# leggedrobotics/wild_visual_navigation

Hardware: AMD Instinct MI355X
Metric: frames/sec (448x448 DINO-ViT-S/8 + seg + MLP train-step) (higher is better)
Workload: dtype fp16 + e5m2-MX-correction linears (a w = a_h w_h + 2^-12 (a_h8 w_l8 + a_l8 w_h8); ~16 significand bits per product) + f16 attention products (two-plane q in the first six blocks), fp32 accumulate / residual (<= 1e-3 parity mode)

## Files before the change

include/wvn_hip.h:

```cpp
#ifndef WVN_HIP_H
#define WVN_HIP_H
#include <stddef.h>
#ifdef __cplusplus
extern "C" {
#endif

#define WVN_MAX_DEPTH 32
#define WVN_PREC_F32 0
#define WVN_PREC_BF16 1
#define WVN_PREC_X3 2
#define WVN_PREC_FP8 3
#define WVN_PREC_F16 4

#define WVN_PREC_MIX 5

int wvn_version(void);

#define WVN_VIT_MLP_FUSED 1
#define WVN_VIT_QKV_FUSED 2
#define WVN_VIT_FUSE_ANY_SIZE 4
#define WVN_VIT_NO_PROJ_IN_MLP 8
#define WVN_VIT_NO_LN_HANDOVER 16
#define WVN_VIT_NO_A384_X3 32
#define WVN_VIT_X3_NO_A384 64
// ... 289 lines not shown
int wvn_debug_mlp_x3_frag(const void* xn, const void* xn_lo, const void* W1, const void* W1_lo, const float* b1, void* hid, void* hid_lo,
                          const void* W2p, const float* b2, float* x, int M, int F, long long* dbg1, long long* dbg2, void* stream);
int wvn_debug_gemm_n384_mx(const void* A_h, const void* A_l8, const void* A_h8, const void* Wp, const float* bias, const float* ls, float* C,
                           int ldc, int M, int K, long long* dbg, void* stream);
int wvn_debug_mlp_mx(const float* x, int ldx, const float* ln_stats, const float* ln_g, const float* ln_b, const void* W1p, const float* b1,
                     void* hid_h, void* hid_l8, void* hid_h8, const void* W2p, const float* b2, float* xout, int M, int F, long long* dbg1,
                     long long* dbg2, void* stream);
int wvn_debug_qkv_mx(const float* x, int ldx, const float* ln_stats, const float* ln_g, const float* ln_b, const void* Wp, const float* bias, void* q,
                     void* q_lo, void* k, void* vt, int heads, int npad, int ntok_s, float q_scale, int M, long long* dbg, void* stream);
int wvn_debug_f16_saturate(const float* in, void* out_f16, int n, void* stream);
int wvn_debug_attention_timing(long long* dbg);
int wvn_debug_attention_variant(int variant);
int wvn_debug_attention_planes(const void* q, const void* q_lo, const void* k, const void* vt, void* out, void* out_lo, int B, int heads,
                               int ntok, int ntok_s, int npad, int out_frag, int qsplit_form, void* stream);
int wvn_debug_n384_pair(int on);
int wvn_debug_kmeans_assign_form(int form);
int wvn_debug_kmeans_linear_rows(int rows);

int wvn_debug_kmeans_screen_stats(unsigned long long* out, int reset);
int wvn_debug_qkv_fused_timing(long long* dbg);
int wvn_debug_mlp_fused_timing(long long* dbg);
int wvn_debug_gemm_n384(const void* A, int lda, const void* W, int ldw, const float* bias, float* C, int ldc, int M, int K,
                        void* stream);


size_t wvn_dense_crf_workspace_bytes(int B, int H, int W, int K);
int wvn_dense_crf(const float* logits1, int K1, long long s1b, long long s1c, long long s1p, const float* logits2, int K2, long long s2b,
                  long long s2c, long long s2p, const unsigned char* image, int B, int H, int W, int iterations, float pos_w, float pos_xy_std,
                  float bi_w, float bi_xy_std, float bi_rgb_std, int* labels, int* nseg_last, float* probs, float* debug, void* workspace,
                  size_t workspace_bytes, void* stream);
// ... 19 lines not shown
```

wild_visual_navigation_amd/_lib.py:

```python
import ctypes as C
import os
import threading

import torch

_HERE = os.path.dirname(os.path.abspath(__file__))
LIB_PATH = os.environ.get("WVN_LIB_PATH") or os.path.join(_HERE, "lib", "libwvn_hip.so")
if os.environ.get("WVN_LIB_PATH"):
    import sys as _sys

    print(f"[wild_visual_navigation_amd] WVN_LIB_PATH is set: loading {LIB_PATH} instead of the in-tree build", file=_sys.stderr)

WVN_MAX_DEPTH = 32
PREC_F32, PREC_BF16, PREC_X3, PREC_FP8, PREC_F16, PREC_MIX = 0, 1, 2, 3, 4, 5
VIT_MLP_FUSED = 1
VIT_QKV_FUSED = 2
VIT_FUSE_ANY_SIZE = 4
VIT_NO_PROJ_IN_MLP = 8
VIT_NO_LN_HANDOVER = 16
VIT_NO_A384_X3 = 32
VIT_NO_MX = 1024


def vit_qsplit_blocks(n: int) -> int:
# ... 118 lines not shown
    "wvn_slic_connectivity_scratch_bytes": ([_i, _i, _i, _i], _sz),
    "wvn_slic_connectivity": ([_p, _p, _i, _i, _i, _i, _i, _p, _sz, _p], _i),
    "wvn_seg_centers": ([_p, _p, _p, _i, _i, _i, _p], _i),
    "wvn_seg_adjacency": ([_p, _p, _p, _p, _i, _i, _i, _i, _p], _i),
    "wvn_normalize_rows": ([_p, _i, _p, _i, _i, _p], _i),
    "wvn_argmax_rows": ([_p, _i, _i, _i, _p, _p], _i),
    "wvn_kmeans_scratch_bytes": ([_i, _i, _i, _i], _sz),
    "wvn_kmeans_pixels_scratch_bytes": ([_i, _i, _i, _i, _i], _sz),
    "wvn_kmeans_cosine_pixels": ([_p, _p, _p, _p, _i, _i, _i, _i, _i, _i, _i, _p], _i),
    "wvn_flip_average": ([_p, _p, _p, _i, _i, _i, _p], _i),
    "wvn_kmeans_pixels_linear_supported_shape": ([_i, _i, _i, _i], _i),
    "wvn_kmeans_pixels_linear_scratch_bytes": ([_i, _i, _i, _i, _i], _sz),
    "wvn_kmeans_cosine_pixels_linear": ([_p, _p, _p, _p, _i, _i, _i, _i, _i, _i, _i, _p], _i),
    "wvn_debug_kmeans_linear_rows": ([_i], _i),
    "wvn_debug_n384_pair": ([_i], _i),
    "wvn_table_argmax_slots": ([_i], _i),
    "wvn_table_bilerp_argmax": ([_p, _p, _i, _i, _i, _i, _p], _i),
    "wvn_table_bilerp_argmax_ac": ([_p, _p, _i, _i, _i, _i, _i, _p], _i),
    "wvn_kmeans_cosine_pixels_linear_ac": ([_p, _p, _p, _p, _i, _i, _i, _i, _i, _i, _i, _i, _p], _i),
    "wvn_cast_rows": ([_p, _i, _p, _i, _i, _i, _i, _p], _i),
    "wvn_kmeans_cosine": ([_p, _p, _p, _p, _i, _i, _i, _i, _i, _i, _p], _i),
    "wvn_mlp_param_count": ([_p], _sz),
    "wvn_mlp_workspace_bytes": ([_p, _i], _sz),
    "wvn_double_mlp_row_tile": ([], _i),
    "wvn_double_mlp_fused_ok": ([_p, _i], _i),
    "wvn_mlp_forward": ([_p, _p, _p, _i, _i, _p, _p, _p, _p, _sz, _p], _i),
    "wvn_mlp_train_phase_a": ([_p, _p, _p, _i, _p, _i, _p, _p, _sz, _p], _i),
    "wvn_mlp_train_phase_b": ([_p, _p, _p, _i, _p, _p, _i, _p, _f, _f, _f, _p, _p, _p, _sz, _p], _i),
    "wvn_compact_segment_rows": ([_p, _i, _p, _i, _p, _i, _i, _p, _p, _p, _p], _i),
    "wvn_mlp_train_phase_a_rows": ([_p, _p, _p, _i, _p, _i, _p, _p, _p, _sz, _p, _p], _i),
# ... 67 lines not shown
```

wild_visual_navigation_amd/csrc/api.hip:

```cpp
#include <math.h>
#include <string.h>

#include "../../include/wvn_hip.h"

#include "common.h"
#include "wvn_internal.h"

#define RET_IF(x)            \
  do {                       \
    int rc__ = (x);          \
    if (rc__ != WVN_OK) return rc__; \
  } while (0)

extern "C" {

int wvn_version(void) { return 100; }

size_t wvn_vit_workspace_bytes(const wvn_vit_model* m, int batch) {
  if (!m || batch <= 0) return 0;
  return wvn_vit_workspace_bytes_impl(m, batch);
}

int wvn_vit_forward(const wvn_vit_model* m, const float* img, int batch, float* tokens_f32, void* tokens_lowp,
                    int ld_lowp, void* workspace, size_t workspace_bytes, void* stream) {
// ... 214 lines not shown
  if (!W2p) return WVN_OK;
  return wvn_gemm_n384_mx_launch(wvn_desc_n384(hid_h, hid_l8, F, W2p, nullptr, b2, nullptr, xout, 384, M, F, nullptr, dbg2, hid_h8), EPI_RESID_F32, (hipStream_t)stream);
}
int wvn_debug_qkv_mx(const float* x, int ldx, const float* ln_stats, const float* ln_g, const float* ln_b, const void* Wp, const float* bias, void* q,
                     void* q_lo, void* k, void* vt, int heads, int npad, int ntok_s, float q_scale, int M, long long* dbg, void* stream) {
  GemmBf16Params p = wvn_desc_a384(nullptr, nullptr, 0, Wp, nullptr, bias, nullptr, nullptr, 0, M, 3 * heads * 64, dbg);
  wvn_desc_ln_on_load(p, x, ldx, ln_stats, ln_g, ln_b);
  wvn_desc_qkv_epilogue(p, q, k, vt, heads, npad, 0, ntok_s, q_scale, 1, q_lo);
  return wvn_gemm_a384_mx_launch(p, EPI_QKV, (hipStream_t)stream);
}
int wvn_debug_n384_pair(int on) {
  if (on >= 32) { wvn_gemm_a384_mx_set_form(on - 32); return WVN_OK; }
  wvn_gemm_n384_x3_set_pair(on);
  return WVN_OK;
}
int wvn_debug_kmeans_screen_stats(unsigned long long* out, int reset) { return out ? wvn_kmeans_pixels_screen_stats(out, reset) : WVN_ERR_ARG; }
int wvn_debug_kmeans_assign_form(int form) { wvn_kmeans_pixels_set_assign_form(form); return WVN_OK; }
int wvn_debug_attention_variant(int v) { wvn_attention_bf16_set_variant(v); wvn_attention_bf16_set_variant_f16(v); return WVN_OK; }
int wvn_debug_attention_planes(const void* q, const void* q_lo, const void* k, const void* vt, void* out, void* out_lo, int B, int heads, int ntok,
                               int ntok_s, int npad, int out_frag, int qsplit_form, void* stream) {
  if (!q || !k || !vt || !out || B < 1 || heads < 1 || ntok < 1 || ntok_s < ntok || ntok_s > npad) return WVN_ERR_ARG;
  if (qsplit_form < 0 || qsplit_form > 2 || (qsplit_form == 0) != (q_lo == nullptr)) return WVN_ERR_ARG;
  if (out_frag < 0 || out_frag > 2 || (out_frag != 0 && (!out_lo || heads != 6))) return WVN_ERR_ARG;
  return wvn_attention_bf16_launch_f16((const bf16_t*)q, (const bf16_t*)k, (const bf16_t*)vt, (bf16_t*)out, B, heads, ntok, ntok_s, npad, 0.f,
                                       (hipStream_t)stream, (bf16_t*)out_lo, (const bf16_t*)q_lo, out_frag, qsplit_form);
}

int wvn_debug_gemm_bf16_timed(const void* A, int lda, const void* W, int ldw, const float* bias, void* C, int ldc, int M,
                              int N, int K, int epi, long long* dbg, void* stream) {
  if (epi < 0 || epi > EPI_ACCUM_F32 || !C) return WVN_ERR_ARG;
// ... 516 lines not shown
```

wild_visual_navigation_amd/csrc/gemm_n384_x3.hip:

```cpp
#include <type_traits>

#include "common.h"
#include "wvn_internal.h"

namespace {

constexpr int NN = 384;
constexpr int NTILE = NN / 32;
constexpr int BKS = 16;
constexpr int BM = 128;
constexpr int NS = 4;
constexpr int W_PLANE = NN * BKS * 2;
constexpr int A_PLANE = BM * BKS * 2;
constexpr int A_OFF = 2 * W_PLANE;
constexpr int STAGE_BYTES = 2 * W_PLANE + 2 * A_PLANE;
constexpr int RING_BYTES = NS * STAGE_BYTES;
constexpr int STG_PITCH = 132;
constexpr int STG_BYTES = 32 * STG_PITCH * 4;
constexpr int BIAS_OFF = RING_BYTES;
constexpr int LS_OFF = BIAS_OFF + NN * 4;
constexpr int LDS_BYTES = LS_OFF + NN * 4;
constexpr int WP = 6, AP = 2;

struct N384X3Params {
  const bf16_t* A; size_t a_plane; int lda;
  const bf16_t* W; size_t w_plane; int ldw;
  const float* bias; const float* ls;
  float* C; int ldc;
  int M, K;
  long long* dbg;
  float* stats; float eps;
  const float* pos; int npatch, ntok_s, c_rows;
};

__device__ inline void n384_epilogue(const f32x16_t (&acc)[NTILE], unsigned char* smem, int wave, int lane, int m0w, __amdgpu_buffer_rsrc_t rs_c,
                                     int ldc, const float* bias_l, const float* ls_l, float* stats = nullptr, float eps = 0.f, int M = 0,
                                     const float* pos = nullptr, int npatch = 0, int ntok_s = 0) {
  const int l31 = lane & 31, hi = lane >> 5;
  __syncthreads();
  float* stg = (float*)(smem + wave * STG_BYTES);
  const unsigned cvoff = (unsigned)(((lane >> 5) * ldc + (lane & 31) * 4) * 4);
  float s1[16], s2[16];
#pragma unroll
  for (int it = 0; it < 16; ++it) { s1[it] = 0.f; s2[it] = 0.f; }
#pragma unroll
  for (int c = 0; c < 3; ++c) {
#pragma unroll
// ... 314 lines not shown
    }
  }
}

constexpr int PFW = 3;
constexpr int PNS = 6;
constexpr int PRING_BYTES = PNS * FSTAGE;
constexpr int PSTG_PITCH = 68;
constexpr int PSTG_BYTES = 32 * PSTG_PITCH * 4;
constexpr int PBIAS_OFF = PRING_BYTES;
constexpr int PLS_OFF = PBIAS_OFF + NN * 4;
constexpr int PSTAT_OFF = PLS_OFF + NN * 4;
constexpr int PAIR_LDS_BYTES = PSTAT_OFF + 2 * BM * 8;
static_assert(8 * PSTG_BYTES <= PRING_BYTES && PAIR_LDS_BYTES <= 160 * 1024, "staging images must fit in the ring, the whole in the LDS");

__device__ inline void n384_pair_epilogue(const f32x16_t (&acc)[NTILE / 2], unsigned char* smem, int wave, int lane, int rg, int ch, int m0w,
                                          __amdgpu_buffer_rsrc_t rs_c, int ldc, const float* bias_l, const float* ls_l, float* stats, float eps, int M) {
  const int l31 = lane & 31, hi = lane >> 5, l15 = lane & 15, rq = lane >> 4;
  __syncthreads();
  float* stg = (float*)(smem + wave * PSTG_BYTES);
  const unsigned cvoff = (unsigned)((rq * ldc + l15 * 4) * 4);
  const int col0 = 192 * ch;
  float s1[8], s2[8];
#pragma unroll
  for (int it = 0; it < 8; ++it) { s1[it] = 0.f; s2[it] = 0.f; }
#pragma unroll
  for (int c = 0; c < 3; ++c) {
#pragma unroll
    for (int tt = 0; tt < 2; ++tt)
#pragma unroll
      for (int g = 0; g < 4; ++g) {
        const f32x16_t& a = acc[2 * c + tt];
        const f32x4_t o = {a[4 * g], a[4 * g + 1], a[4 * g + 2], a[4 * g + 3]};
        *(f32x4_t*)(stg + l31 * PSTG_PITCH + 32 * tt + 8 * g + 4 * hi) = o;
      }
    const f32x4_t b4 = *(const f32x4_t*)(bias_l + col0 + 64 * c + l15 * 4);
    const f32x4_t l4 = *(const f32x4_t*)(ls_l + col0 + 64 * c + l15 * 4);
    u32x4_t r[8];
    unsigned so_dst[8];
#pragma unroll
    for (int it = 0; it < 8; ++it) {
      so_dst[it] = __builtin_amdgcn_readfirstlane(((m0w + 4 * it) * ldc + col0 + 64 * c) * 4);
      r[it] = __builtin_amdgcn_raw_buffer_load_b128(rs_c, cvoff, so_dst[it], 0);
    }
#pragma unroll
    for (int it = 0; it < 8; ++it) {
      const f32x4_t v = *(const f32x4_t*)(stg + (4 * it + rq) * PSTG_PITCH + l15 * 4);
      u32x4_t o;
#pragma unroll
      for (int e = 0; e < 4; ++e) {
        const float y = (v[e] + b4[e]) * l4[e] + __uint_as_float(r[it][e]);
        o[e] = __float_as_uint(y);
        s1[it] += y;
        s2[it] = fmaf(y, y, s2[it]);
      }
      wvn_store_b128_guarded(o, rs_c, cvoff, so_dst[it]);
    }
  }
  if (stats) {
    float* sx = (float*)(smem + PSTAT_OFF);
    auto dpp_add = [](float v, auto ctrl) {
      constexpr int C = decltype(ctrl)::value;
      return v + __builtin_bit_cast(float, __builtin_amdgcn_update_dpp(0, __builtin_bit_cast(int, v), C, 0xf, 0xf, false));
    };
#pragma unroll
    for (int it = 0; it < 8; ++it) {
      float a = s1[it], b = s2[it];
      a = dpp_add(a, std::integral_constant<int, 0xB1>{}); b = dpp_add(b, std::integral_constant<int, 0xB1>{});
      a = dpp_add(a, std::integral_constant<int, 0x4E>{}); b = dpp_add(b, std::integral_constant<int, 0x4E>{});
      a = dpp_add(a, std::integral_constant<int, 0x141>{}); b = dpp_add(b, std::integral_constant<int, 0x141>{});
      a = dpp_add(a, std::integral_constant<int, 0x140>{}); b = dpp_add(b, std::integral_constant<int, 0x140>{});
      if (l15 == 0) *(wvn_f32x2_t*)(sx + ((size_t)ch * BM + rg * 32 + 4 * it + rq) * 2) = wvn_f32x2_t{a, b};
    }
    __syncthreads();
    if (ch == 0 && lane < 32) {
      const int m = m0w + lane;
      if (m < M) {
        const wvn_f32x2_t p0 = *(const wvn_f32x2_t*)(sx + ((size_t)rg * 32 + lane) * 2), p1 = *(const wvn_f32x2_t*)(sx + ((size_t)BM + rg * 32 + lane) * 2);
        const float a = p0[0] + p1[0], b = p0[1] + p1[1];
        const float mean = a * (1.0f / NN);
        const float var = fmaxf(b * (1.0f / NN) - mean * mean, 0.f);
        *(wvn_f32x2_t*)(stats + 2 * (size_t)m) = wvn_f32x2_t{mean, 1.0f / sqrtf(var + eps)};
      }
    }
  }
}

template <bool TIMING>
__global__ __launch_bounds__(512, 1) void gemm_n384_x3_frag_pair_kernel(N384X3Params p) {
  wvn_fp16_saturate();
  extern __shared__ __attribute__((aligned(16))) unsigned char smem[];
  const int tid = threadIdx.x, lane = tid & 63;
  const int wave = __builtin_amdgcn_readfirstlane(tid >> 6);
  const int rg = wave & 3, ch = wave >> 2;
  const int l31 = lane & 31, hi = lane >> 5;
  const int nk = p.K / BKS;
  const float* bias_l = (const float*)(smem + PBIAS_OFF);
  const float* ls_l = (const float*)(smem + PLS_OFF);
  for (int i = tid; i < NN; i += 512) {
    ((float*)(smem + PBIAS_OFF))[i] = p.bias ? p.bias[i] : 0.f;
    ((float*)(smem + PLS_OFF))[i] = p.ls ? p.ls[i] : 1.f;
  }
  const __amdgpu_buffer_rsrc_t rs_w = __builtin_amdgcn_make_buffer_rsrc((void*)p.W, 0, (unsigned)((size_t)2 * NN * p.K * 2), 0x00020000);
  const size_t mpad = (size_t)(p.M + 31) / 32 * 32;
  const __amdgpu_buffer_rsrc_t rs_a = __builtin_amdgcn_make_buffer_rsrc((void*)p.A, 0, (unsigned)((p.a_plane + mpad * p.K) * 2), 0x00020000);
  const __amdgpu_buffer_rsrc_t rs_c = __builtin_amdgcn_make_buffer_rsrc((void*)p.C, 0, (unsigned)((size_t)p.M * p.ldc * 4), 0x00020000);
  const unsigned wv0 = (unsigned)(wave * PFW * 1024 + lane * 16);
  const unsigned rdw = l31 * 32 + ((hi ^ ((l31 >> 3) & 1)) << 4) + ch * 6 * 1024;
  const unsigned a_lo_off = (unsigned)(p.a_plane * 2);

  long long t_wait = 0, t_steps = 0, t_epi = 0;
  const long long t_start = TIMING ? (long long)__builtin_amdgcn_s_memtime() : 0;
  const int nrb = (p.M + BM - 1) / BM;
  for (int rb = blockIdx.x; rb < nrb; rb += gridDim.x) {
    const int m0w = rb * BM + rg * 32;
    const unsigned a_base = __builtin_amdgcn_readfirstlane((unsigned)((size_t)(m0w >> 5) * nk * 1024));
    auto piece_w = [&](int i, int u) {
      unsigned char* st = smem + (i % PNS) * FSTAGE;
      __builtin_amdgcn_raw_ptr_buffer_load_lds(rs_w, (__attribute__((address_space(3))) void*)(st + (wave * PFW + u) * 1024), 16, wv0 + u * 1024,
                                               __builtin_amdgcn_readfirstlane((unsigned)i * FSTAGE), 0, 0);
    };
    u32x4_t afh[PD], afl[PD];
    auto load_a = [&](int i, int slot) {
      const unsigned so = __builtin_amdgcn_readfirstlane(a_base + (unsigned)i * 1024);
      afh[slot] = __builtin_amdgcn_raw_buffer_load_b128(rs_a, lane * 16, so, 0);
      afl[slot] = __builtin_amdgcn_raw_buffer_load_b128(rs_a, lane * 16, so + a_lo_off, 0);
    };
    __syncthreads();
#pragma unroll
    for (int j = 0; j < PD; ++j) load_a(j, j);
#pragma unroll
    for (int i0 = 0; i0 < PNS - 1; ++i0)
      if (i0 < nk) {
#pragma unroll
        for (int u = 0; u < PFW; ++u) piece_w(i0, u);
      }

    f32x16_t acc[NTILE / 2];
#pragma unroll
    for (int t = 0; t < NTILE / 2; ++t)
#pragma unroll
      for (int r = 0; r < 16; ++r) acc[t][r] = 0.f;

    bf16x8_t wh[2][2], wl[2][2];
    asm volatile("s_waitcnt vmcnt(%0)" ::"n"((PNS - 2) * PFW) : "memory");
    __builtin_amdgcn_s_barrier();
#pragma unroll
    for (int t = 0; t < 2; ++t) {
      wh[0][t] = *(const bf16x8_t*)(smem + rdw + t * 1024);
      wl[0][t] = *(const bf16x8_t*)(smem + rdw + W_PLANE + t * 1024);
    }
    for (int ib = 0; ib < nk; ib += PD) {
#pragma unroll
      for (int jj = 0; jj < PD; ++jj) {
        const int i = ib + jj;
        long long c0 = 0, c1 = 0;
        if constexpr (TIMING) c0 = (long long)__builtin_amdgcn_s_memtime();
        asm volatile("s_waitcnt vmcnt(%0)" ::"n"((PNS - 3) * PFW) : "memory");
        __builtin_amdgcn_s_barrier();
        if constexpr (TIMING) c1 = (long long)__builtin_amdgcn_s_memtime();
        __builtin_amdgcn_sched_barrier(0);
// ... 37 lines not shown
        }
        if (i + PD < nk) load_a(i + PD, jj);
        __builtin_amdgcn_sched_barrier(0);
        if constexpr (TIMING) { t_wait += c1 - c0; t_steps += (long long)__builtin_amdgcn_s_memtime() - c1; }
      }
    }
    long long e0 = 0;
    if constexpr (TIMING) e0 = (long long)__builtin_amdgcn_s_memtime();
    asm volatile("s_waitcnt vmcnt(0)" ::: "memory");
    n384_pair_epilogue(acc, smem, wave, lane, rg, ch, m0w, rs_c, p.ldc, bias_l, ls_l, p.stats, p.eps, p.M);
    if constexpr (TIMING) t_epi += (long long)__builtin_amdgcn_s_memtime() - e0;
  }
  if constexpr (TIMING) {
    if (lane == 0 && p.dbg && ch == 0) {
      long long* d = p.dbg + ((size_t)blockIdx.x * 4 + rg) * 4;
      d[0] = t_wait; d[1] = t_steps; d[2] = t_epi; d[3] = (long long)__builtin_amdgcn_s_memtime() - t_start;
    }
  }
}

typedef __attribute__((ext_vector_type(8))) int i32x8_t;
typedef __attribute__((ext_vector_type(8))) _Float16 f16x8_t;
constexpr int MXD = 2;
constexpr int MX_SC_ONE = 0x7f7f7f7f, MX_SC_RES = 0x73737373;

struct N384MXExtra { unsigned a_l8_off; };

template <bool TIMING, int VAR = 0>
__global__ __launch_bounds__(512, 1) void gemm_n384_mx_pair_kernel(N384X3Params p, N384MXExtra ex) {
  wvn_fp16_saturate();
  extern __shared__ __attribute__((aligned(16))) unsigned char smem[];
  const int tid = threadIdx.x, lane = tid & 63;
  const int wave = __builtin_amdgcn_readfirstlane(tid >> 6);
  const int rg = wave & 3, ch = wave >> 2;
  const int l31 = lane & 31, hi = lane >> 5;
  const int nk = p.K / BKS;
  const int nmac = p.K / 64;
  const float* bias_l = (const float*)(smem + PBIAS_OFF);
  const float* ls_l = (const float*)(smem + PLS_OFF);
  for (int i = tid; i < NN; i += 512) {
    ((float*)(smem + PBIAS_OFF))[i] = p.bias ? p.bias[i] : 0.f;
    ((float*)(smem + PLS_OFF))[i] = p.ls ? p.ls[i] : 1.f;
  }
  const __amdgpu_buffer_rsrc_t rs_w = __builtin_amdgcn_make_buffer_rsrc((void*)p.W, 0, (unsigned)((size_t)4 * NN * p.K), 0x00020000);
  const size_t mpad = (size_t)(p.M + 31) / 32 * 32;
  const __amdgpu_buffer_rsrc_t rs_a = __builtin_amdgcn_make_buffer_rsrc((void*)p.A, 0, (unsigned)(ex.a_l8_off + mpad * p.K), 0x00020000);
  const __amdgpu_buffer_rsrc_t rs_c = __builtin_amdgcn_make_buffer_rsrc((void*)p.C, 0, (unsigned)((size_t)p.M * p.ldc * 4), 0x00020000);
  const unsigned wv0 = (unsigned)(wave * PFW * 1024 + lane * 16);
  const unsigned rdw = l31 * 32 + ((hi ^ ((l31 >> 3) & 1)) << 4) + ch * 6 * 1024;

  long long t_wait = 0, t_steps = 0, t_epi = 0;
  const long long t_start = TIMING ? (long long)__builtin_amdgcn_s_memtime() : 0;
  const int nrb = (p.M + BM - 1) / BM;
  for (int rb = blockIdx.x; rb < nrb; rb += gridDim.x) {
    const int m0w = rb * BM + rg * 32;
    const unsigned a_base = __builtin_amdgcn_readfirstlane((unsigned)((size_t)(m0w >> 5) * p.K * 64));
    const unsigned a8_base = __builtin_amdgcn_readfirstlane((unsigned)((size_t)(m0w >> 5) * p.K * 32));
    auto piece_w = [&](int i, int u) {
      unsigned char* st = smem + (i % PNS) * FSTAGE;
      __builtin_amdgcn_raw_ptr_buffer_load_lds(rs_w, (__attribute__((address_space(3))) void*)(st + (wave * PFW + u) * 1024), 16, wv0 + u * 1024,
                                               __builtin_amdgcn_readfirstlane((unsigned)i * FSTAGE), 0, 0);
    };
    u32x4_t ah[MXD][4], a8[MXD][2][2];
    auto load_ah = [&](int c, int slot) {
#pragma unroll
      for (int s = 0; s < 4; ++s)
// ... 9 lines not shown
      typedef __attribute__((ext_vector_type(2))) _Float16 h2_t;
#pragma unroll
      for (int sfr = 0; sfr < 4; ++sfr) {
        uint32_t d[2] = {0, 0};
#pragma unroll
        for (int e = 0; e < 4; ++e) {
          const uint32_t pr = ah[slot][sfr][e];
          const s16x2_t o = __builtin_bit_cast(s16x2_t, d[e >> 1]);
          d[e >> 1] = __builtin_bit_cast(uint32_t, (e & 1) ? __builtin_amdgcn_cvt_scalef32_pk_bf8_f16(o, __builtin_bit_cast(h2_t, pr), 1.0f, true)
                                                           : __builtin_amdgcn_cvt_scalef32_pk_bf8_f16(o, __builtin_bit_cast(h2_t, pr), 1.0f, false));
        }
        a8[slot][0][sfr >> 1][2 * (sfr & 1)] = d[0];
        a8[slot][0][sfr >> 1][2 * (sfr & 1) + 1] = d[1];
      }
    };
    __syncthreads();
#pragma unroll
    for (int c = 0; c < MXD; ++c) {
      load_ah(c, c);
      __builtin_amdgcn_sched_barrier(0);
      load_a8(c, c);
      __builtin_amdgcn_sched_barrier(0);
    }
#pragma unroll
    for (int i0 = 0; i0 < PNS - 1; ++i0)
      if (i0 < nk) {
#pragma unroll
        for (int u = 0; u < PFW; ++u) piece_w(i0, u);
      }

    f32x16_t acc[NTILE / 2];
#pragma unroll
    for (int t = 0; t < NTILE / 2; ++t)
#pragma unroll
      for (int r = 0; r < 16; ++r) acc[t][r] = 0.f;

    u32x4_t wq[2][2][2];
    asm volatile("s_waitcnt vmcnt(%0)" ::"n"((PNS - 2) * PFW) : "memory");
    __builtin_amdgcn_s_barrier();
#pragma unroll
    for (int x = 0; x < 2; ++x)
#pragma unroll
      for (int t = 0; t < 2; ++t) wq[0][x][t] = *(const u32x4_t*)(smem + rdw + x * W_PLANE + t * 1024);
    for (int ib = 0; ib < nk; ib += 4 * MXD) {
#pragma unroll
      for (int jj = 0; jj < 4 * MXD; ++jj) {
        const int i = ib + jj;
        const int kind = jj & 3, slot = jj >> 2;
        long long c0 = 0, c1 = 0;
        if constexpr (TIMING) c0 = (long long)__builtin_amdgcn_s_memtime();
        if constexpr (VAR != 4) {
          constexpr int W3 = (PNS - 3) * PFW;
          if (jj == 0) { if (i == 0) asm volatile("s_waitcnt vmcnt(%0)" ::"n"(W3) : "memory"); else asm volatile("s_waitcnt vmcnt(%0)" ::"n"(W3 + 6) : "memory"); }
          else if (jj == 1) { if (i == 1) asm volatile("s_waitcnt vmcnt(%0)" ::"n"(W3) : "memory"); else asm volatile("s_waitcnt vmcnt(%0)" ::"n"(W3 + 2) : "memory"); }
          else if (jj == 2) { if (i == 2) asm volatile("s_waitcnt vmcnt(%0)" ::"n"(W3 + 4) : "memory"); else asm volatile("s_waitcnt vmcnt(%0)" ::"n"(W3 + 6) : "memory"); }
          else if ((jj & 3) == 0) asm volatile("s_waitcnt vmcnt(%0)" ::"n"(W3 + 6) : "memory");
          else if ((jj & 3) == 1) asm volatile("s_waitcnt vmcnt(%0)" ::"n"(W3 + 2) : "memory");
          else if ((jj & 3) == 2) asm volatile("s_waitcnt vmcnt(%0)" ::"n"(W3 + 6) : "memory");
          else asm volatile("s_waitcnt vmcnt(%0)" ::"n"(W3 + 4) : "memory");
// ... 38 lines not shown
              acc[2 * pr + t] = __builtin_amdgcn_mfma_scale_f32_32x32x64_f8f6f4(wv, av, acc[2 * pr + t], 1, 1, 0, kind == 2 ? MX_SC_RES : MX_SC_ONE, 0,
                                                                                kind == 2 ? MX_SC_ONE : MX_SC_RES);
            }
#pragma unroll
            for (int n = 0; n < 2; ++n) {
              __builtin_amdgcn_sched_group_barrier(0x008, 1, 0);
              __builtin_amdgcn_sched_group_barrier(0x100, 2, 0);
              __builtin_amdgcn_sched_group_barrier(0x010, 1, 0);
              __builtin_amdgcn_sched_group_barrier(0x002, 4, 0);
            }
          }
          __builtin_amdgcn_sched_barrier(0);
        }
        const int c2 = (i >> 2) + MXD;
        if constexpr (!(VAR & 2) || VAR == 4) {
          if (kind == 1) load_ah(c2, slot);
          if (kind == 3) load_a8(c2, slot);
        }
        __builtin_amdgcn_sched_barrier(0);
        if constexpr (TIMING) { t_wait += c1 - c0; t_steps += (long long)__builtin_amdgcn_s_memtime() - c1; }
      }
    }
    long long e0 = 0;
    if constexpr (TIMING) e0 = (long long)__builtin_amdgcn_s_memtime();
    asm volatile("s_waitcnt vmcnt(0)" ::: "memory");
    n384_pair_epilogue(acc, smem, wave, lane, rg, ch, m0w, rs_c, p.ldc, bias_l, ls_l, p.stats, p.eps, p.M);
    if constexpr (TIMING) t_epi += (long long)__builtin_amdgcn_s_memtime() - e0;
  }
  if constexpr (TIMING) {
    if (lane == 0 && p.dbg && ch == 0) {
      long long* d = p.dbg + ((size_t)blockIdx.x * 4 + rg) * 4;
      d[0] = t_wait; d[1] = t_steps; d[2] = t_epi; d[3] = (long long)__builtin_amdgcn_s_memtime() - t_start;
    }
  }
}

int g_n384_mx_var = 0;
int g_n384_pair = 1;

int n384x3_num_cus() {
  static int n = 0;
  if (n == 0) {
    int dev = 0;
    hipDeviceProp_t prop;
    if (hipGetDevice(&dev) == hipSuccess && hipGetDeviceProperties(&prop, dev) == hipSuccess) n = prop.multiProcessorCount;
    if (n <= 0) n = 256;
  }
  return n;
}

}

// ... 21 lines not shown
  else hipLaunchKernelGGL(gemm_n384_x3_kernel<false>, dim3(grid), dim3(256), LDS_BYTES, st, p);
  WVN_LAUNCH_CHECK();
  return WVN_OK;
}

int wvn_gemm_n384_x3_frag_launch(const GemmBf16Params& g, int epi, hipStream_t st) {
  if (epi != EPI_RESID_F32 && epi != EPI_ACCUM_F32) return WVN_ERR_ARG;
  if (g.N != NN || g.K <= 0 || (g.K % (BKS * PD)) != 0 || g.M <= 0 || !g.A || !g.A_lo || !g.W || !g.C || (g.ldc % 4)) return WVN_ERR_ARG;
  if (((uintptr_t)g.A | (uintptr_t)g.A_lo | (uintptr_t)g.W | (uintptr_t)g.C) & 15) return WVN_ERR_ARG;
  if (g.A_lo <= g.A) return WVN_ERR_ARG;
  const size_t a_plane = (size_t)(g.A_lo - g.A), mpad = (size_t)(g.M + 31) / 32 * 32;
  if ((a_plane + mpad * g.K) * 2 >= (1ull << 32) || (size_t)g.M * g.ldc * 4 >= (1ull << 32) || (size_t)2 * NN * g.K * 2 >= (1ull << 31)) return WVN_ERR_ARG;
  N384X3Params p{};
  p.A = g.A; p.a_plane = a_plane; p.lda = g.K; p.W = g.W; p.w_plane = 0; p.ldw = g.K; p.bias = g.bias; p.ls = g.ls;
  p.C = (float*)g.C; p.ldc = g.ldc; p.M = g.M; p.K = g.K; p.dbg = g.dbg; p.stats = g.ln_stats_out; p.eps = g.ln_eps;
  static LdsOptIn lds_opt_in;
  if (const int rc = lds_opt_in(PAIR_LDS_BYTES, (const void*)gemm_n384_x3_frag_kernel<false>, (const void*)gemm_n384_x3_frag_kernel<true>,
                                (const void*)gemm_n384_x3_frag_pair_kernel<false>, (const void*)gemm_n384_x3_frag_pair_kernel<true>)) return rc;
  const int ncu = n384x3_num_cus(), nrb = ceil_div(g.M, BM);
  const int grid = nrb < ncu ? nrb : ncu;
  if (g_n384_pair) {
    if (p.dbg) hipLaunchKernelGGL(gemm_n384_x3_frag_pair_kernel<true>, dim3(grid), dim3(512), PAIR_LDS_BYTES, st, p);
    else hipLaunchKernelGGL(gemm_n384_x3_frag_pair_kernel<false>, dim3(grid), dim3(512), PAIR_LDS_BYTES, st, p);
  } else if (p.dbg) hipLaunchKernelGGL(gemm_n384_x3_frag_kernel<true>, dim3(grid), dim3(256), LDS_BYTES, st, p);
  else hipLaunchKernelGGL(gemm_n384_x3_frag_kernel<false>, dim3(grid), dim3(256), LDS_BYTES, st, p);
  WVN_LAUNCH_CHECK();
  return WVN_OK;
}
int wvn_gemm_n384_mx_launch(const GemmBf16Params& g, int epi, hipStream_t st) {
  if (epi != EPI_RESID_F32 && epi != EPI_ACCUM_F32) return WVN_ERR_ARG;
  if (g.N != NN || g.K <= 0 || (g.K % 128) != 0 || g.M <= 0 || !g.A || !g.A_lo || !g.W || !g.C || (g.ldc % 4)) return WVN_ERR_ARG;
  if (((uintptr_t)g.A | (uintptr_t)g.A_lo | (uintptr_t)g.W | (uintptr_t)g.C) & 15) return WVN_ERR_ARG;
  const size_t mpad = (size_t)(g.M + 31) / 32 * 32;
  const uintptr_t a0 = (uintptr_t)g.A, al = (uintptr_t)g.A_lo;
  if (al < a0 + mpad * g.K * 2) return WVN_ERR_ARG;
  const uintptr_t top = al + mpad * g.K;
  if (top - a0 >= (1ull << 32) || (size_t)g.M * g.ldc * 4 >= (1ull << 32) || (size_t)4 * NN * g.K >= (1ull << 31)) return WVN_ERR_ARG;
  N384X3Params p{};
  p.A = g.A; p.a_plane = 0; p.lda = g.K; p.W = g.W; p.w_plane = 0; p.ldw = g.K; p.bias = g.bias; p.ls = g.ls;
  p.C = (float*)g.C; p.ldc = g.ldc; p.M = g.M; p.K = g.K; p.dbg = g.dbg; p.stats = g.ln_stats_out; p.eps = g.ln_eps;
  N384MXExtra ex{(unsigned)(al - a0)};
  static LdsOptIn lds_opt_in;
  if (const int rc = lds_opt_in(PAIR_LDS_BYTES, (const void*)gemm_n384_mx_pair_kernel<false>, (const void*)gemm_n384_mx_pair_kernel<true>,
                                (const void*)gemm_n384_mx_pair_kernel<true, 1>, (const void*)gemm_n384_mx_pair_kernel<true, 2>,
                                (const void*)gemm_n384_mx_pair_kernel<true, 3>, (const void*)gemm_n384_mx_pair_kernel<true, 4>)) return rc;
  const int ncu = n384x3_num_cus(), nrb = ceil_div(g.M, BM);
  const int grid = nrb < ncu ? nrb : ncu;
  if (p.dbg && g_n384_mx_var == 1) hipLaunchKernelGGL((gemm_n384_mx_pair_kernel<true, 1>), dim3(grid), dim3(512), PAIR_LDS_BYTES, st, p, ex);
  else if (p.dbg && g_n384_mx_var == 2) hipLaunchKernelGGL((gemm_n384_mx_pair_kernel<true, 2>), dim3(grid), dim3(512), PAIR_LDS_BYTES, st, p, ex);
  else if (p.dbg && g_n384_mx_var == 3) hipLaunchKernelGGL((gemm_n384_mx_pair_kernel<true, 3>), dim3(grid), dim3(512), PAIR_LDS_BYTES, st, p, ex);
  else if (p.dbg && g_n384_mx_var == 4) hipLaunchKernelGGL((gemm_n384_mx_pair_kernel<true, 4>), dim3(grid), dim3(512), PAIR_LDS_BYTES, st, p, ex);
  else if (p.dbg) hipLaunchKernelGGL(gemm_n384_mx_pair_kernel<true>, dim3(grid), dim3(512), PAIR_LDS_BYTES, st, p, ex);
  else hipLaunchKernelGGL(gemm_n384_mx_pair_kernel<false>, dim3(grid), dim3(512), PAIR_LDS_BYTES, st, p, ex);
  WVN_LAUNCH_CHECK();
  return WVN_OK;
}
void wvn_gemm_n384_x3_set_pair(int on) {
  if (on >= 16) { g_n384_mx_var = on - 16; return; }
  g_n384_pair = on ? 1 : 0;
}
```

wild_visual_navigation_amd/csrc/wvn_internal.h:

```cpp
#pragma once
#include "common.h"

enum GemmEpilogue {
  EPI_BF16 = 0,
  EPI_GELU_BF16 = 1,
  EPI_RELU_BF16 = 2,
  EPI_F32 = 3,
  EPI_RESID_F32 = 4,
  EPI_ACCUM_F32 = 5,
  EPI_PATCH = 6,
  EPI_QKV = 7,
  EPI_GELU_MX8 = 9,
  EPI_GELU_FRAG = 8,
};

struct GemmBf16Params {
  const bf16_t* A; int lda;
  const bf16_t* W; int ldw;
  const float* bias;
  void* C; int ldc;
  int M, N, K;
  const float* pos; int npatch; int ntok;
  int ntok_s;
  bf16_t* q; bf16_t* k; bf16_t* vt; int heads; int npad;
// ... 144 lines not shown
int wvn_normalize_rows_launch(const float* code, int ldc, float* xn, int rows, int C, hipStream_t st);
int wvn_argmax_rows_launch(const float* x, int ld, int rows, int cols, int* out, hipStream_t st);
size_t wvn_kmeans_scratch_floats(int B, int P, int C, int K);
size_t wvn_kmeans_pixels_scratch_floats(int B, int G, int H, int C, int K);
int wvn_kmeans_pixels_launch(const float* code, int* labels, int* nseg, float* scratch, int B, int G, int H, int C, int K, int iters,
                             int relabel, hipStream_t st);
int wvn_km_pix_prepare_launch(const float* code, float* rinv, float* cent, int B, int G, int H, int C, int K, hipStream_t st, int align_corners = 1);
int wvn_km_relabel_launch(int* labels, int* nseg, int B, long long P, int K, int relabel, hipStream_t st);
int wvn_kmeans_pixels_linear_supported(int G, int H, int C, int K);
size_t wvn_kmeans_pixels_linear_scratch_floats(int B, int G, int H, int C, int K);
void wvn_kmeans_pixels_linear_set_rows(int rc);
int wvn_kmeans_pixels_linear_launch(const float* code, int* labels, int* nseg, float* scratch, int B, int G, int H, int C, int K,
                                    int iters, int relabel, hipStream_t st, int align_corners = 1);
int wvn_f16_saturate_probe_launch(const float* in, uint16_t* out, int n, hipStream_t st);
void wvn_gemm_n384_x3_set_pair(int on);
void wvn_gemm_a384_mx_set_form(int form);
int wvn_table_slots(int K);
int wvn_table_bilerp_argmax_launch(const float* table, int* labels, int B, int G, int H, int K, hipStream_t st, int align_corners = 1);
void wvn_kmeans_pixels_set_assign_form(int form);
int wvn_kmeans_pixels_screen_stats(unsigned long long* out, int reset);
int wvn_flip_average_launch(const float* a, const float* mirrored, float* out, int B, int G, int C, hipStream_t st);
int wvn_kmeans_launch(const float* xn, int* labels, int* nseg, float* scratch, int B, int P, int C, int K, int iters,
                      int relabel, hipStream_t st);
struct ConfArgs {
  int method = 0;
  int balanced = 1;
  double* state = nullptr;
  float* minmax = nullptr;
};
int wvn_mlp_rowloss_stats_launch(const float* out, int ldo, const float* x, int ldx, const unsigned char* valid,
// ... 101 lines not shown
```

Before: 883.0.

## Prefetch residual tile into freed A registers during last K-step of n384 MX GEMM

In the final K iteration of the N=384 MX pair GEMM, the freed A-operand prefetch registers are reused to issue residual (C) loads instead of further A loads. The new early epilogue then loads only the remaining quads, waits, and applies bias, layer-scale and residual, storing all 24 quads together. The goal is to hide residual-read latency behind the last MFMA steps rather than leaving it exposed at the start of the epilogue. It raises register pressure and makes the wait counts and register aliasing fragile. It also adds prologue timing instrumentation and a debug or env switch, with the new form on by default.

```diff
diff --git a/include/wvn_hip.h b/include/wvn_hip.h
--- a/include/wvn_hip.h
+++ b/include/wvn_hip.h
@@ -327,6 +327,7 @@
 int wvn_debug_attention_planes(const void* q, const void* q_lo, const void* k, const void* vt, void* out, void* out_lo, int B, int heads,
                                int ntok, int ntok_s, int npad, int out_frag, int qsplit_form, void* stream);
 int wvn_debug_n384_pair(int on);
+int wvn_debug_n384_epilogue(int form, int time_prologue);
 int wvn_debug_kmeans_assign_form(int form);
 int wvn_debug_kmeans_linear_rows(int rows);
 
diff --git a/wild_visual_navigation_amd/_lib.py b/wild_visual_navigation_amd/_lib.py
--- a/wild_visual_navigation_amd/_lib.py
+++ b/wild_visual_navigation_amd/_lib.py
@@ -156,6 +156,7 @@
     "wvn_kmeans_cosine_pixels_linear": ([_p, _p, _p, _p, _i, _i, _i, _i, _i, _i, _i, _p], _i),
     "wvn_debug_kmeans_linear_rows": ([_i], _i),
     "wvn_debug_n384_pair": ([_i], _i),
+    "wvn_debug_n384_epilogue": ([_i, _i], _i),
     "wvn_table_argmax_slots": ([_i], _i),
     "wvn_table_bilerp_argmax": ([_p, _p, _i, _i, _i, _i, _p], _i),
     "wvn_table_bilerp_argmax_ac": ([_p, _p, _i, _i, _i, _i, _i, _p], _i),
diff --git a/wild_visual_navigation_amd/csrc/api.hip b/wild_visual_navigation_amd/csrc/api.hip
--- a/wild_visual_navigation_amd/csrc/api.hip
+++ b/wild_visual_navigation_amd/csrc/api.hip
@@ -252,6 +252,7 @@
   wvn_gemm_n384_x3_set_pair(on);
   return WVN_OK;
 }
+int wvn_debug_n384_epilogue(int form, int time_prologue) { return wvn_gemm_n384_x3_set_epilogue(form, time_prologue); }
 int wvn_debug_kmeans_screen_stats(unsigned long long* out, int reset) { return out ? wvn_kmeans_pixels_screen_stats(out, reset) : WVN_ERR_ARG; }
 int wvn_debug_kmeans_assign_form(int form) { wvn_kmeans_pixels_set_assign_form(form); return WVN_OK; }
 int wvn_debug_attention_variant(int v) { wvn_attention_bf16_set_variant(v); wvn_attention_bf16_set_variant_f16(v); return WVN_OK; }
diff --git a/wild_visual_navigation_amd/csrc/gemm_n384_x3.hip b/wild_visual_navigation_amd/csrc/gemm_n384_x3.hip
--- a/wild_visual_navigation_amd/csrc/gemm_n384_x3.hip
+++ b/wild_visual_navigation_amd/csrc/gemm_n384_x3.hip
@@ -31,6 +31,7 @@
   long long* dbg;
   float* stats; float eps;
   const float* pos; int npatch, ntok_s, c_rows;
+  int dbg_prologue;
 };
 
 __device__ inline void n384_epilogue(const f32x16_t (&acc)[NTILE], unsigned char* smem, int wave, int lane, int m0w, __amdgpu_buffer_rsrc_t rs_c,
@@ -375,6 +376,53 @@
 constexpr int PAIR_LDS_BYTES = PSTAT_OFF + 2 * BM * 8;
 static_assert(8 * PSTG_BYTES <= PRING_BYTES && PAIR_LDS_BYTES <= 160 * 1024, "staging images must fit in the ring, the whole in the LDS");
 
+constexpr int RQ = 24;
+
+__device__ inline void n384_pair_stage(const f32x16_t (&acc)[NTILE / 2], float* stg, int c, int l31, int hi) {
+#pragma unroll
+  for (int tt = 0; tt < 2; ++tt)
+#pragma unroll
+    for (int g = 0; g < 4; ++g) {
+      const f32x16_t& a = acc[2 * c + tt];
+      const f32x4_t o = {a[4 * g], a[4 * g + 1], a[4 * g + 2], a[4 * g + 3]};
+      *(f32x4_t*)(stg + l31 * PSTG_PITCH + 32 * tt + 8 * g + 4 * hi) = o;
+    }
+}
+
+__device__ inline unsigned n384_pair_quad_soff(int q, int m0w, int ldc, int col0) {
+  return __builtin_amdgcn_readfirstlane(((m0w + 4 * (q & 7)) * ldc + col0 + 64 * (q >> 3)) * 4);
+}
+
+__device__ inline void n384_pair_stats(const float (&s1)[8], const float (&s2)[8], unsigned char* smem, int lane, int rg, int ch, int m0w, float* stats,
+                                       float eps, int M) {
+  const int l15 = lane & 15, rq = lane >> 4;
+  float* sx = (float*)(smem + PSTAT_OFF);
+  auto dpp_add = [](float v, auto ctrl) {
+    constexpr int C = decltype(ctrl)::value;
+    return v + __builtin_bit_cast(float, __builtin_amdgcn_update_dpp(0, __builtin_bit_cast(int, v), C, 0xf, 0xf, false));
+  };
+#pragma unroll
+  for (int it = 0; it < 8; ++it) {
+    float a = s1[it], b = s2[it];
+    a = dpp_add(a, std::integral_constant<int, 0xB1>{}); b = dpp_add(b, std::integral_constant<int, 0xB1>{});
+    a = dpp_add(a, std::integral_constant<int, 0x4E>{}); b = dpp_add(b, std::integral_constant<int, 0x4E>{});
+    a = dpp_add(a, std::integral_constant<int, 0x141>{}); b = dpp_add(b, std::integral_constant<int, 0x141>{});
+    a = dpp_add(a, std::integral_constant<int, 0x140>{}); b = dpp_add(b, std::integral_constant<int, 0x140>{});
+    if (l15 == 0) *(wvn_f32x2_t*)(sx + ((size_t)ch * BM + rg * 32 + 4 * it + rq) * 2) = wvn_f32x2_t{a, b};
+  }
+  __syncthreads();
+  if (ch == 0 && lane < 32) {
+    const int m = m0w + lane;
+    if (m < M) {
+      const wvn_f32x2_t p0 = *(const wvn_f32x2_t*)(sx + ((size_t)rg * 32 + lane) * 2), p1 = *(const wvn_f32x2_t*)(sx + ((size_t)BM + rg * 32 + lane) * 2);
+      const float a = p0[0] + p1[0], b = p0[1] + p1[1];
+      const float mean = a * (1.0f / NN);
+      const float var = fmaxf(b * (1.0f / NN) - mean * mean, 0.f);
+      *(wvn_f32x2_t*)(stats + 2 * (size_t)m) = wvn_f32x2_t{mean, 1.0f / sqrtf(var + eps)};
+    }
+  }
+}
+
 __device__ inline void n384_pair_epilogue(const f32x16_t (&acc)[NTILE / 2], unsigned char* smem, int wave, int lane, int rg, int ch, int m0w,
                                           __amdgpu_buffer_rsrc_t rs_c, int ldc, const float* bias_l, const float* ls_l, float* stats, float eps, int M) {
   const int l31 = lane & 31, hi = lane >> 5, l15 = lane & 15, rq = lane >> 4;
@@ -387,21 +435,14 @@
   for (int it = 0; it < 8; ++it) { s1[it] = 0.f; s2[it] = 0.f; }
 #pragma unroll
   for (int c = 0; c < 3; ++c) {
-#pragma unroll
-    for (int tt = 0; tt < 2; ++tt)
-#pragma unroll
-      for (int g = 0; g < 4; ++g) {
-        const f32x16_t& a = acc[2 * c + tt];
-        const f32x4_t o = {a[4 * g], a[4 * g + 1], a[4 * g + 2], a[4 * g + 3]};
-        *(f32x4_t*)(stg + l31 * PSTG_PITCH + 32 * tt + 8 * g + 4 * hi) = o;
-      }
+    n384_pair_stage(acc, stg, c, l31, hi);
     const f32x4_t b4 = *(const f32x4_t*)(bias_l + col0 + 64 * c + l15 * 4);
     const f32x4_t l4 = *(const f32x4_t*)(ls_l + col0 + 64 * c + l15 * 4);
     u32x4_t r[8];
     unsigned so_dst[8];
 #pragma unroll
     for (int it = 0; it < 8; ++it) {
-      so_dst[it] = __builtin_amdgcn_readfirstlane(((m0w + 4 * it) * ldc + col0 + 64 * c) * 4);
+      so_dst[it] = n384_pair_quad_soff(8 * c + it, m0w, ldc, col0);
       r[it] = __builtin_amdgcn_raw_buffer_load_b128(rs_c, cvoff, so_dst[it], 0);
     }
 #pragma unroll
@@ -418,33 +459,50 @@
       wvn_store_b128_guarded(o, rs_c, cvoff, so_dst[it]);
     }
   }
-  if (stats) {
-    float* sx = (float*)(smem + PSTAT_OFF);
-    auto dpp_add = [](float v, auto ctrl) {
-      constexpr int C = decltype(ctrl)::value;
-      return v + __builtin_bit_cast(float, __builtin_amdgcn_update_dpp(0, __builtin_bit_cast(int, v), C, 0xf, 0xf, false));
-    };
+  if (stats) n384_pair_stats(s1, s2, smem, lane, rg, ch, m0w, stats, eps, M);
+}
+
+template <int FIRST>
+__device__ inline void n384_pair_epilogue_early(const f32x16_t (&acc)[NTILE / 2], u32x4_t (&r)[RQ], unsigned char* smem, int wave, int lane, int rg, int ch,
+                                                int m0w, __amdgpu_buffer_rsrc_t rs_c, int ldc, const float* bias_l, const float* ls_l, float* stats, float eps,
+                                                int M) {
+  asm volatile("" : "+v"(lane));
+  const int l31 = lane & 31, hi = lane >> 5, l15 = lane & 15, rq = lane >> 4;
+  float* stg = (float*)(smem + wave * PSTG_BYTES);
+  const unsigned cvoff = (unsigned)((rq * ldc + l15 * 4) * 4);
+  const int col0 = 192 * ch;
+#pragma unroll
+  for (int q = FIRST; q < RQ; ++q) r[q] = __builtin_amdgcn_raw_buffer_load_b128(rs_c, cvoff, n384_pair_quad_soff(q, m0w, ldc, col0), 0);
+  __builtin_amdgcn_sched_barrier(0);
+  asm volatile("s_waitcnt vmcnt(%0) lgkmcnt(0)" ::"n"(RQ - FIRST) : "memory");
+  __builtin_amdgcn_s_barrier();
+  __builtin_amdgcn_sched_barrier(0);
+  float s1[8], s2[8];
+#pragma unroll
+  for (int it = 0; it < 8; ++it) { s1[it] = 0.f; s2[it] = 0.f; }
+#pragma unroll
+  for (int c = 0; c < 3; ++c) {
+    n384_pair_stage(acc, stg, c, l31, hi);
+    const f32x4_t b4 = *(const f32x4_t*)(bias_l + col0 + 64 * c + l15 * 4);
+    const f32x4_t l4 = *(const f32x4_t*)(ls_l + col0 + 64 * c + l15 * 4);
 #pragma unroll
     for (int it = 0; it < 8; ++it) {
-      float a = s1[it], b = s2[it];
-      a = dpp_add(a, std::integral_constant<int, 0xB1>{}); b = dpp_add(b, std::integral_constant<int, 0xB1>{});
-      a = dpp_add(a, std::integral_constant<int, 0x4E>{}); b = dpp_add(b, std::integral_constant<int, 0x4E>{});
-      a = dpp_add(a, std::integral_constant<int, 0x141>{}); b = dpp_add(b, std::integral_constant<int, 0x141>{});
-      a = dpp_add(a, std::integral_constant<int, 0x140>{}); b = dpp_add(b, std::integral_constant<int, 0x140>{});
-      if (l15 == 0) *(wvn_f32x2_t*)(sx + ((size_t)ch * BM + rg * 32 + 4 * it + rq) * 2) = wvn_f32x2_t{a, b};
-    }
-    __syncthreads();
-    if (ch == 0 && lane < 32) {
-      const int m = m0w + lane;
-      if (m < M) {
-        const wvn_f32x2_t p0 = *(const wvn_f32x2_t*)(sx + ((size_t)rg * 32 + lane) * 2), p1 = *(const wvn_f32x2_t*)(sx + ((size_t)BM + rg * 32 + lane) * 2);
-        const float a = p0[0] + p1[0], b = p0[1] + p1[1];
-        const float mean = a * (1.0f / NN);
-        const float var = fmaxf(b * (1.0f / NN) - mean * mean, 0.f);
-        *(wvn_f32x2_t*)(stats + 2 * (size_t)m) = wvn_f32x2_t{mean, 1.0f / sqrtf(var + eps)};
-      }
-    }
-  }
+      const f32x4_t v = *(const f32x4_t*)(stg + (4 * it + rq) * PSTG_PITCH + l15 * 4);
+      u32x4_t o;
+#pragma unroll
+      for (int e = 0; e < 4; ++e) {
+        const float y = (v[e] + b4[e]) * l4[e] + __uint_as_float(r[8 * c + it][e]);
+        o[e] = __float_as_uint(y);
+        s1[it] += y;
+        s2[it] = fmaf(y, y, s2[it]);
+      }
+      r[8 * c + it] = o;
+    }
+  }
+  __builtin_amdgcn_sched_barrier(0);
+#pragma unroll
+  for (int q = 0; q < RQ; ++q) wvn_store_b128_guarded(r[q], rs_c, cvoff, n384_pair_quad_soff(q, m0w, ldc, col0));
+  if (stats) n384_pair_stats(s1, s2, smem, lane, rg, ch, m0w, stats, eps, M);
 }
 
 template <bool TIMING>
@@ -470,7 +528,7 @@
   const unsigned rdw = l31 * 32 + ((hi ^ ((l31 >> 3) & 1)) << 4) + ch * 6 * 1024;
   const unsigned a_lo_off = (unsigned)(p.a_plane * 2);
 
-  long long t_wait = 0, t_steps = 0, t_epi = 0;
+  long long t_wait = 0, t_steps = 0, t_epi = 0, t_pro = 0;
   const long long t_start = TIMING ? (long long)__builtin_amdgcn_s_memtime() : 0;
   const int nrb = (p.M + BM - 1) / BM;
   for (int rb = blockIdx.x; rb < nrb; rb += gridDim.x) {
@@ -487,6 +545,8 @@
       afh[slot] = __builtin_amdgcn_raw_buffer_load_b128(rs_a, lane * 16, so, 0);
       afl[slot] = __builtin_amdgcn_raw_buffer_load_b128(rs_a, lane * 16, so + a_lo_off, 0);
     };
+    long long p0 = 0;
+    if constexpr (TIMING) p0 = (long long)__builtin_amdgcn_s_memtime();
     __syncthreads();
 #pragma unroll
     for (int j = 0; j < PD; ++j) load_a(j, j);
@@ -506,6 +566,7 @@
     bf16x8_t wh[2][2], wl[2][2];
     asm volatile("s_waitcnt vmcnt(%0)" ::"n"((PNS - 2) * PFW) : "memory");
     __builtin_amdgcn_s_barrier();
+    if constexpr (TIMING) t_pro += (long long)__builtin_amdgcn_s_memtime() - p0;
 #pragma unroll
     for (int t = 0; t < 2; ++t) {
       wh[0][t] = *(const bf16x8_t*)(smem + rdw + t * 1024);
@@ -573,19 +634,20 @@
   if constexpr (TIMING) {
     if (lane == 0 && p.dbg && ch == 0) {
       long long* d = p.dbg + ((size_t)blockIdx.x * 4 + rg) * 4;
-      d[0] = t_wait; d[1] = t_steps; d[2] = t_epi; d[3] = (long long)__builtin_amdgcn_s_memtime() - t_start;
+      d[0] = p.dbg_prologue ? t_pro : t_wait; d[1] = t_steps; d[2] = t_epi; d[3] = (long long)__builtin_amdgcn_s_memtime() - t_start;
     }
   }
 }
 
 typedef __attribute__((ext_vector_type(8))) int i32x8_t;
 typedef __attribute__((ext_vector_type(8))) _Float16 f16x8_t;
+constexpr int N384_EPILOGUE_DEFAULT = 1;
 constexpr int MXD = 2;
 constexpr int MX_SC_ONE = 0x7f7f7f7f, MX_SC_RES = 0x73737373;
 
 struct N384MXExtra { unsigned a_l8_off; };
 
-template <bool TIMING, int VAR = 0>
+template <bool TIMING, int VAR = 0, int FORM = 0>
 __global__ __launch_bounds__(512, 1) void gemm_n384_mx_pair_kernel(N384X3Params p, N384MXExtra ex) {
   wvn_fp16_saturate();
   extern __shared__ __attribute__((aligned(16))) unsigned char smem[];
@@ -608,7 +670,7 @@
   const unsigned wv0 = (unsigned)(wave * PFW * 1024 + lane * 16);
   const unsigned rdw = l31 * 32 + ((hi ^ ((l31 >> 3) & 1)) << 4) + ch * 6 * 1024;
 
-  long long t_wait = 0, t_steps = 0, t_epi = 0;
+  long long t_wait = 0, t_steps = 0, t_epi = 0, t_pro = 0;
   const long long t_start = TIMING ? (long long)__builtin_amdgcn_s_memtime() : 0;
   const int nrb = (p.M + BM - 1) / BM;
   for (int rb = blockIdx.x; rb < nrb; rb += gridDim.x) {
@@ -648,6 +710,8 @@
         a8[slot][0][sfr >> 1][2 * (sfr & 1) + 1] = d[1];
       }
     };
+    long long p0 = 0;
+    if constexpr (TIMING) p0 = (long long)__builtin_amdgcn_s_memtime();
     __syncthreads();
 #pragma unroll
     for (int c = 0; c < MXD; ++c) {
@@ -672,11 +736,20 @@
     u32x4_t wq[2][2][2];
     asm volatile("s_waitcnt vmcnt(%0)" ::"n"((PNS - 2) * PFW) : "memory");
     __builtin_amdgcn_s_barrier();
+    if constexpr (TIMING) t_pro += (long long)__builtin_amdgcn_s_memtime() - p0;
 #pragma unroll
     for (int x = 0; x < 2; ++x)
 #pragma unroll
       for (int t = 0; t < 2; ++t) wq[0][x][t] = *(const u32x4_t*)(smem + rdw + x * W_PLANE + t * 1024);
+    auto load_res = [&](int q0, int n, u32x4_t* dst) {
+      int l = lane;
+      asm volatile("" : "+v"(l));
+      const unsigned cvoff_r = (unsigned)(((l >> 4) * p.ldc + (l & 15) * 4) * 4);
+#pragma unroll
+      for (int j = 0; j < n; ++j) dst[j] = __builtin_amdgcn_raw_buffer_load_b128(rs_c, cvoff_r, n384_pair_quad_soff(q0 + j, m0w, p.ldc, 192 * ch), 0);
+    };
     for (int ib = 0; ib < nk; ib += 4 * MXD) {
+      const bool last = FORM == 1 && ib + 4 * MXD >= nk;
 #pragma unroll
       for (int jj = 0; jj < 4 * MXD; ++jj) {
         const int i = ib + jj;
@@ -745,8 +818,13 @@
         }
         const int c2 = (i >> 2) + MXD;
         if constexpr (!(VAR & 2) || VAR == 4) {
-          if (kind == 1) load_ah(c2, slot);
-          if (kind == 3) load_a8(c2, slot);
+          if (last) {
+            if (kind == 1) load_res(6 * slot, 4, ah[slot]);
+            if (kind == 3) load_res(6 * slot + 4, 2, a8[slot][1]);
+          } else {
+            if (kind == 1) load_ah(c2, slot);
+            if (kind == 3) load_a8(c2, slot);
+          }
         }
         __builtin_amdgcn_sched_barrier(0);
         if constexpr (TIMING) { t_wait += c1 - c0; t_steps += (long long)__builtin_amdgcn_s_memtime() - c1; }
@@ -754,19 +832,34 @@
     }
     long long e0 = 0;
     if constexpr (TIMING) e0 = (long long)__builtin_amdgcn_s_memtime();
-    asm volatile("s_waitcnt vmcnt(0)" ::: "memory");
-    n384_pair_epilogue(acc, smem, wave, lane, rg, ch, m0w, rs_c, p.ldc, bias_l, ls_l, p.stats, p.eps, p.M);
+    if constexpr (FORM == 0) {
+      asm volatile("s_waitcnt vmcnt(0)" ::: "memory");
+      n384_pair_epilogue(acc, smem, wave, lane, rg, ch, m0w, rs_c, p.ldc, bias_l, ls_l, p.stats, p.eps, p.M);
+    } else {
+      u32x4_t res[RQ];
+#pragma unroll
+      for (int sl = 0; sl < MXD; ++sl) {
+#pragma unroll
+        for (int s = 0; s < 4; ++s) res[6 * sl + s] = ah[sl][s];
+#pragma unroll
+        for (int x = 0; x < 2; ++x) res[6 * sl + 4 + x] = a8[sl][1][x];
+      }
+      n384_pair_epilogue_early<6 * MXD>(acc, res, smem, wave, lane, rg, ch, m0w, rs_c, p.ldc, bias_l, ls_l, p.stats, p.eps, p.M);
+    }
     if constexpr (TIMING) t_epi += (long long)__builtin_amdgcn_s_memtime() - e0;
   }
   if constexpr (TIMING) {
     if (lane == 0 && p.dbg && ch == 0) {
       long long* d = p.dbg + ((size_t)blockIdx.x * 4 + rg) * 4;
-      d[0] = t_wait; d[1] = t_steps; d[2] = t_epi; d[3] = (long long)__builtin_amdgcn_s_memtime() - t_start;
+      d[0] = p.dbg_prologue ? t_pro : t_wait; d[1] = t_steps; d[2] = t_epi; d[3] = (long long)__builtin_amdgcn_s_memtime() - t_start;
     }
   }
 }
 
 int g_n384_mx_var = 0;
+int g_n384_epilogue = [] { const char* e = getenv("WVN_N384_EPILOGUE"); return e && (e[0] == '0' || e[0] == '1') && !e[1] ? e[0] - '0' : N384_EPILOGUE_DEFAULT; }();
+const int g_n384_epilogue_initial = g_n384_epilogue;
+int g_n384_dbg_prologue = 0;
 int g_n384_pair = 1;
 
 int n384x3_num_cus() {
@@ -818,6 +911,7 @@
   N384X3Params p{};
   p.A = g.A; p.a_plane = a_plane; p.lda = g.K; p.W = g.W; p.w_plane = 0; p.ldw = g.K; p.bias = g.bias; p.ls = g.ls;
   p.C = (float*)g.C; p.ldc = g.ldc; p.M = g.M; p.K = g.K; p.dbg = g.dbg; p.stats = g.ln_stats_out; p.eps = g.ln_eps;
+  p.dbg_prologue = g_n384_dbg_prologue;
   static LdsOptIn lds_opt_in;
   if (const int rc = lds_opt_in(PAIR_LDS_BYTES, (const void*)gemm_n384_x3_frag_kernel<false>, (const void*)gemm_n384_x3_frag_kernel<true>,
                                 (const void*)gemm_n384_x3_frag_pair_kernel<false>, (const void*)gemm_n384_x3_frag_pair_kernel<true>)) return rc;
@@ -843,22 +937,32 @@
   N384X3Params p{};
   p.A = g.A; p.a_plane = 0; p.lda = g.K; p.W = g.W; p.w_plane = 0; p.ldw = g.K; p.bias = g.bias; p.ls = g.ls;
   p.C = (float*)g.C; p.ldc = g.ldc; p.M = g.M; p.K = g.K; p.dbg = g.dbg; p.stats = g.ln_stats_out; p.eps = g.ln_eps;
+  p.dbg_prologue = g_n384_dbg_prologue;
   N384MXExtra ex{(unsigned)(al - a0)};
   static LdsOptIn lds_opt_in;
   if (const int rc = lds_opt_in(PAIR_LDS_BYTES, (const void*)gemm_n384_mx_pair_kernel<false>, (const void*)gemm_n384_mx_pair_kernel<true>,
                                 (const void*)gemm_n384_mx_pair_kernel<true, 1>, (const void*)gemm_n384_mx_pair_kernel<true, 2>,
-                                (const void*)gemm_n384_mx_pair_kernel<true, 3>, (const void*)gemm_n384_mx_pair_kernel<true, 4>)) return rc;
+                                (const void*)gemm_n384_mx_pair_kernel<true, 3>, (const void*)gemm_n384_mx_pair_kernel<true, 4>,
+                                (const void*)gemm_n384_mx_pair_kernel<false, 0, 1>, (const void*)gemm_n384_mx_pair_kernel<true, 0, 1>)) return rc;
   const int ncu = n384x3_num_cus(), nrb = ceil_div(g.M, BM);
   const int grid = nrb < ncu ? nrb : ncu;
   if (p.dbg && g_n384_mx_var == 1) hipLaunchKernelGGL((gemm_n384_mx_pair_kernel<true, 1>), dim3(grid), dim3(512), PAIR_LDS_BYTES, st, p, ex);
   else if (p.dbg && g_n384_mx_var == 2) hipLaunchKernelGGL((gemm_n384_mx_pair_kernel<true, 2>), dim3(grid), dim3(512), PAIR_LDS_BYTES, st, p, ex);
   else if (p.dbg && g_n384_mx_var == 3) hipLaunchKernelGGL((gemm_n384_mx_pair_kernel<true, 3>), dim3(grid), dim3(512), PAIR_LDS_BYTES, st, p, ex);
   else if (p.dbg && g_n384_mx_var == 4) hipLaunchKernelGGL((gemm_n384_mx_pair_kernel<true, 4>), dim3(grid), dim3(512), PAIR_LDS_BYTES, st, p, ex);
+  else if (p.dbg && g_n384_epilogue == 1) hipLaunchKernelGGL((gemm_n384_mx_pair_kernel<true, 0, 1>), dim3(grid), dim3(512), PAIR_LDS_BYTES, st, p, ex);
   else if (p.dbg) hipLaunchKernelGGL(gemm_n384_mx_pair_kernel<true>, dim3(grid), dim3(512), PAIR_LDS_BYTES, st, p, ex);
+  else if (g_n384_epilogue == 1) hipLaunchKernelGGL((gemm_n384_mx_pair_kernel<false, 0, 1>), dim3(grid), dim3(512), PAIR_LDS_BYTES, st, p, ex);
   else hipLaunchKernelGGL(gemm_n384_mx_pair_kernel<false>, dim3(grid), dim3(512), PAIR_LDS_BYTES, st, p, ex);
   WVN_LAUNCH_CHECK();
   return WVN_OK;
 }
+int wvn_gemm_n384_x3_set_epilogue(int form, int time_prologue) {
+  if (form < -1 || form > 1) return WVN_ERR_ARG;
+  g_n384_epilogue = form < 0 ? g_n384_epilogue_initial : form;
+  g_n384_dbg_prologue = time_prologue ? 1 : 0;
+  return WVN_OK;
+}
 void wvn_gemm_n384_x3_set_pair(int on) {
   if (on >= 16) { g_n384_mx_var = on - 16; return; }
   g_n384_pair = on ? 1 : 0;
diff --git a/wild_visual_navigation_amd/csrc/wvn_internal.h b/wild_visual_navigation_amd/csrc/wvn_internal.h
--- a/wild_visual_navigation_amd/csrc/wvn_internal.h
+++ b/wild_visual_navigation_amd/csrc/wvn_internal.h
@@ -182,6 +182,7 @@
                                     int iters, int relabel, hipStream_t st, int align_corners = 1);
 int wvn_f16_saturate_probe_launch(const float* in, uint16_t* out, int n, hipStream_t st);
 void wvn_gemm_n384_x3_set_pair(int on);
+int wvn_gemm_n384_x3_set_epilogue(int form, int time_prologue);
 void wvn_gemm_a384_mx_set_form(int form);
 int wvn_table_slots(int K);
 int wvn_table_bilerp_argmax_launch(const float* table, int* labels, int B, int G, int H, int K, hipStream_t st, int align_corners = 1);
```

After: 888.0, median of 6. About the same (+0.6%).
